# stevenlsw/reart

Measured on AMD Instinct MI355X. Metric: relaxation-loop iterations/sec, higher is better.
Workload: dtype f32; 1 GPU; synthetic T=20 x N=4096, P=20, Chamfer+flow, full iteration, one instance/GPU; frames=20, points=4096, parts=20, flow=True, graph=True, steps_per_graph=20, graph_replays=1, eager_steps=0, parallelism=instances x1, instances_per_gpu=1

## Files before the change

### reart_amd/csrc/prune.hip

```cpp
#include "common.h"
#include "internal.h"
#include <math.h>
#include <string.h>
#include <stddef.h>

typedef float f2 __attribute__((ext_vector_type(2)));
struct SearchHot {
    const float *q, *q_alt, *tsoa, *boxes;
    const int *seed;
    float *pd;
    int *pi;
    unsigned int *cost;
    int P1, Ppad, nqg, P2;
    const int *tlen;
};
static_assert(sizeof(SearchHot) == 88 && offsetof(KnnJob, tlen) == offsetof(SearchHot, tlen) && offsetof(KnnJob, q) == 0 && offsetof(KnnJob, q_alt) == offsetof(SearchHot, q_alt) &&
              offsetof(KnnJob, tsoa) == offsetof(SearchHot, tsoa) && offsetof(KnnJob, boxes) == offsetof(SearchHot, boxes) &&
              offsetof(KnnJob, seed) == offsetof(SearchHot, seed) && offsetof(KnnJob, pd) == offsetof(SearchHot, pd) &&
              offsetof(KnnJob, pi) == offsetof(SearchHot, pi) && offsetof(KnnJob, cost) == offsetof(SearchHot, cost) &&
              offsetof(KnnJob, P1) == offsetof(SearchHot, P1) && offsetof(KnnJob, Ppad) == offsetof(SearchHot, Ppad) &&
              offsetof(KnnJob, nqg) == offsetof(SearchHot, nqg) && offsetof(KnnJob, P2) == offsetof(SearchHot, P2),
              "SearchHot mirrors the head of KnnJob");
__device__ __forceinline__ int pr_uniform_word(const void *p) { return *(const __attribute__((address_space(4))) int *)p; }
#define PR_SMAX 4
#define PR_QCAP 640
#define PR_WPE 6
#define PR_LDS_WAVE_BYTES (64 * 4 + 64 * 16 + 3 * 64 * 8 + PR_QCAP * 4)

#ifdef REART_PRUNE_STATS
__device__ unsigned long long g_prune_stats[8];
extern "C" int reart_debug_prune_stats(unsigned long long *out, int reset) {
    if (hipMemcpyFromSymbol(out, HIP_SYMBOL(g_prune_stats), sizeof(g_prune_stats)) != hipSuccess) return REART_ERR_LAUNCH;
    if (reset) { unsigned long long z[8] = {0}; (void)hipMemcpyToSymbol(HIP_SYMBOL(g_prune_stats), z, sizeof(z)); }
    return REART_OK;
}
#define PRUNE_STAT(k, v) do { if ((threadIdx.x & 63) == 0) atomicAdd(&g_prune_stats[k], (unsigned long long)(v)); } while (0)
#else
#define PRUNE_STAT(k, v) do { } while (0)
#endif
#ifdef REART_PRUNE_PHASE
__device__ unsigned long long g_prune_phase[8];
extern "C" int reart_debug_prune_phase(unsigned long long *out, int reset) {
    if (hipMemcpyFromSymbol(out, HIP_SYMBOL(g_prune_phase), sizeof(g_prune_phase)) != hipSuccess) return REART_ERR_LAUNCH;
    if (reset) { unsigned long long z[8] = {0}; (void)hipMemcpyToSymbol(HIP_SYMBOL(g_prune_phase), z, sizeof(z)); }
    return REART_OK;
}
#define PH_DECL unsigned long long ph_t = __builtin_amdgcn_s_memtime(), ph_acc[7] = {0, 0, 0, 0, 0, 0, 0}
#define PH(k) do { const unsigned long long n_ = __builtin_amdgcn_s_memtime(); ph_acc[k] += n_ - ph_t; ph_t = n_; } while (0)
#define PH_FLUSH(from, to) do { if ((threadIdx.x & 63) == 0) for (int k_ = from; k_ <= to; ++k_) atomicAdd(&g_prune_phase[k_], ph_acc[k_]); } while (0)
__device__ unsigned long long g_prune_head[2][8];
extern "C" int reart_debug_prune_head(unsigned long long *out, int reset) {
    if (hipMemcpyFromSymbol(out, HIP_SYMBOL(g_prune_head), sizeof(g_prune_head)) != hipSuccess) return REART_ERR_LAUNCH;
    if (reset) { unsigned long long z[16] = {0}; (void)hipMemcpyToSymbol(HIP_SYMBOL(g_prune_head), z, sizeof(z)); }
    return REART_OK;
}
#define PH_HEAD_DECL unsigned long long hd_t = ph_t, hd_acc[3] = {0, 0, 0}
#define PH_STAMP(k, ...) do { asm volatile("" :: __VA_ARGS__); const unsigned long long n_ = __builtin_amdgcn_s_memtime(); hd_acc[k] = n_ - hd_t; hd_t = n_; } while (0)
#define PH_HEAD_FLUSH(row) do { if ((threadIdx.x & 63) == 0) { for (int k_ = 0; k_ < 3; ++k_) atomicAdd(&g_prune_head[row][1 + k_], hd_acc[k_]); \
                                atomicAdd(&g_prune_head[row][4], ph_acc[0]); atomicAdd(&g_prune_head[row][6], 1ull); } } while (0)
#define PH_ENTRY const unsigned long long hd_entry = __builtin_amdgcn_s_memtime(); unsigned long long hd_head = 0ull
#define PH_HEAD_END do { hd_head = __builtin_amdgcn_s_memtime() - hd_entry; } while (0)
#define PH_ENTRY_FLUSH(row) do { if ((threadIdx.x & 63) == 0) { atomicAdd(&g_prune_head[row][0], hd_head); \
                                 atomicAdd(&g_prune_head[row][5], __builtin_amdgcn_s_memtime() - hd_entry); } } while (0)
#else
#define PH_DECL do { } while (0)
#define PH(k) do { } while (0)
#define PH_FLUSH(from, to) do { } while (0)
#define PH_HEAD_DECL do { } while (0)
#define PH_STAMP(k, ...) do { } while (0)
#define PH_HEAD_FLUSH(row) do { } while (0)
#define PH_ENTRY do { } while (0)
#define PH_HEAD_END do { } while (0)
#define PH_ENTRY_FLUSH(row) do { } while (0)
#endif

#define PR_WORK(w) ((unsigned)(w) << 20)

#define PR_DPP_OP(NAME, OP, CTRLTXT)                                                                              \
    __device__ __forceinline__ float NAME(float v) {                                                              \
        float r;                                                                                                  \
        asm("s_nop 1\n\t" OP " %0, %1, %1 " CTRLTXT " row_mask:0xf bank_mask:0xf" : "=v"(r) : "v"(v));            \
        return r;                                                                                                 \
    }
PR_DPP_OP(pr_min_q1, "v_min_f32_dpp", "quad_perm:[1,0,3,2]")
PR_DPP_OP(pr_min_q2, "v_min_f32_dpp", "quad_perm:[2,3,0,1]")
PR_DPP_OP(pr_min_hm, "v_min_f32_dpp", "row_half_mirror")
PR_DPP_OP(pr_min_rm, "v_min_f32_dpp", "row_mirror")
PR_DPP_OP(pr_max_q1, "v_max_f32_dpp", "quad_perm:[1,0,3,2]")
PR_DPP_OP(pr_max_q2, "v_max_f32_dpp", "quad_perm:[2,3,0,1]")
PR_DPP_OP(pr_max_hm, "v_max_f32_dpp", "row_half_mirror")
PR_DPP_OP(pr_max_rm, "v_max_f32_dpp", "row_mirror")
__device__ __forceinline__ float pr_row16_min(float v) { return pr_min_rm(pr_min_hm(pr_min_q2(pr_min_q1(v)))); }
__device__ __forceinline__ float pr_row16_max(float v) { return pr_max_rm(pr_max_hm(pr_max_q2(pr_max_q1(v)))); }

__device__ __forceinline__ float rl(float v, int lane) {
    return __int_as_float(__builtin_amdgcn_readlane(__float_as_int(v), lane));
}

__device__ __forceinline__ float box_lb(float lo0, float lo1, float lo2, float hi0, float hi1, float hi2,
                                        float qlo0, float qlo1, float qlo2, float qhi0, float qhi1, float qhi2) {
    const float ex = fmaxf(fmaxf(lo0 - qhi0, qlo0 - hi0), 0.f);
    const float ey = fmaxf(fmaxf(lo1 - qhi1, qlo1 - hi1), 0.f);
    const float ez = fmaxf(fmaxf(lo2 - qhi2, qlo2 - hi2), 0.f);
    return (ex * ex + ey * ey) + ez * ez;
}

template <int KK, bool LDSV, int QCAP, bool BOXL>
__device__ __forceinline__ void knn_pruned_wave(const float *qcloud, const int *seed_p, const int P1, const int n2,
                                                const int S, const int sparse, const int b, const int g,
                                                const int s, const float *cloud, const int cstride, const float *boxes_p,
                                                float *s_tg, float *s_qc, unsigned int *s_q, float *s_bb, const int share, float *s_xthr,
                                                unsigned long long *s_key, float &qx_o, float &qy_o, float &qz_o,
                                                float (&bm)[KK], int (&bb)[KK], int &work_o, unsigned int &pairs_o) {
    struct { int S, sparse; } a = {S, sparse};
    const int lane = threadIdx.x & 63;
    PH_DECL;
    PH_HEAD_DECL;

    const int i = g * NN_BS + lane;
    const int ic = i < P1 ? i : P1 - 1;
    const float *qp = (const float *)((const char *)qcloud + 12u * (unsigned)ic);
    const float qx = qp[0], qy = qp[1], qz = qp[2];
    PH_STAMP(0, "v"(qx), "v"(qy), "v"(qz));
    const f2 qx2 = {qx, qx}, qy2 = {qy, qy}, qz2 = {qz, qz};

    const float *tx = cloud;
    const float *ty = tx + cstride;
    const float *tz = ty + cstride;
    const int nbox = (n2 + NN_BOX - 1) / NN_BOX;
    const float *bx = boxes_p;

    float thr = 0.f;
    unsigned int wp = 0u;
    {
        const int *sd = (const int *)((const char *)(seed_p + (size_t)b * P1 * KK) + 4u * KK * (unsigned)ic);
        int sj[KK];
        bool ok = true;
#pragma unroll
        for (int k = 0; k < KK; ++k) {
            sj[k] = sd[k];
            ok = ok && sj[k] >= 0 && sj[k] < n2;
#pragma unroll
            for (int k2 = 0; k2 < k; ++k2) ok = ok && sj[k] != sj[k2];
        }
        PH_STAMP(1, "v"(sj[0]), "v"(sj[KK - 1]), "s"(n2));
        constexpr bool SCR_JOINT = BOXL;
        constexpr bool SCR_FITS = (384 + QCAP + (SCR_JOINT ? 384 : 0)) >= KK * 3 * 64;
        if (SCR_FITS && share) {
            float *s_scr = (float *)s_key;
            float sx[KK], sy[KK], sz[KK];
#pragma unroll
            for (int k = 0; k < KK; ++k) {
                const int j = ok ? sj[k] : 0;
                sx[k] = tx[j]; sy[k] = ty[j]; sz[k] = tz[j];
            }
            if (!LDSV) __builtin_amdgcn_sched_barrier(0);
#pragma unroll
            for (int k = 0; k < KK; ++k) {
                s_scr[(3 * k + 0) * 64 + lane] = ok ? sx[k] : INFINITY;
                s_scr[(3 * k + 1) * 64 + lane] = ok ? sy[k] : INFINITY;
                s_scr[(3 * k + 2) * 64 + lane] = ok ? sz[k] : INFINITY;
            }
            PH_STAMP(2, "v"(lane));
            thr = INFINITY;
            const float *row = s_scr + (lane & 48);
            const bool split = s_xthr != nullptr && a.S > 1;
            const int c0 = split ? 2 * s : 0, cstep = split ? 2 * a.S : 2;
            wp = 64u * KK * 2u * (unsigned)((16 - c0 + cstep - 1) / cstep);
#pragma unroll 1
            for (int c = c0; c < 16; c += cstep) {
                f2 far = {0.f, 0.f};
#pragma unroll
                for (int k = 0; k < KK; ++k) {
                    const f2 dx = qx2 - *(const f2 *)(row + (3 * k + 0) * 64 + c);
                    const f2 dy = qy2 - *(const f2 *)(row + (3 * k + 1) * 64 + c);
                    const f2 dz = qz2 - *(const f2 *)(row + (3 * k + 2) * 64 + c);
                    const f2 d = (dx * dx + dy * dy) + dz * dz;
                    far = f2{fmaxf(far.x, d.x), fmaxf(far.y, d.y)};
                }
                thr = fminf(thr, fminf(far.x, far.y));
            }
            if (split) {
                s_xthr[64 * s + lane] = thr;
                __syncthreads();
                for (int t = 0; t < a.S; ++t) thr = fminf(thr, s_xthr[64 * t + lane]);
            }
            if (!(qx == qx && qy == qy && qz == qz)) thr = INFINITY;
        } else {
#pragma unroll
            for (int k = 0; k < KK; ++k) {
                const int j = ok ? sj[k] : 0;
                thr = fmaxf(thr, reart_sqdist3(qx, qy, qz, tx[j], ty[j], tz[j]));
            }
            wp = 64u * KK;
            if (!ok || !(thr >= 0.f)) thr = INFINITY;
        }
    }

    const float gl0 = pr_row16_min(qx), gl1 = pr_row16_min(qy), gl2 = pr_row16_min(qz);
    const float gh0 = pr_row16_max(qx), gh1 = pr_row16_max(qy), gh2 = pr_row16_max(qz);
    const float gt = pr_row16_max(thr);
    float G[4][7];
#pragma unroll
    for (int q = 0; q < 4; ++q) {
        G[q][0] = rl(gl0, 16 * q); G[q][1] = rl(gl1, 16 * q); G[q][2] = rl(gl2, 16 * q);
        G[q][3] = rl(gh0, 16 * q); G[q][4] = rl(gh1, 16 * q); G[q][5] = rl(gh2, 16 * q);
        G[q][6] = rl(gt, 16 * q);
    }

#pragma unroll
    for (int k = 0; k < KK; ++k) { bm[k] = INFINITY; bb[k] = -1; }
    const float *tx_g = tx;
    wp |= PR_WORK(16);

    const int queue_max = a.sparse;
    int qcnt = 0;
    ((float4 *)s_qc)[lane] = make_float4(qx, qy, qz, 0.f);
    if (KK == 1) s_key[lane] = ~0ull;
    else { s_key[lane] = ~0ull; s_key[64 + lane] = ~0ull; s_key[128 + lane] = ~0ull; }
    auto drain_queue = [&]() {
        for (int e0 = 0; e0 < qcnt; e0 += 64) {
            wp += PR_WORK(6);
            const int e = e0 + lane;
            const bool valid = e < qcnt;
            const unsigned ent = s_q[valid ? e : e0];
            const int ql = (int)(ent & 63u), j0 = (int)(ent >> 6) * NN_BOX;
            wp += (unsigned)__builtin_popcountll(__ballot(valid)) * NN_BOX;
            const float4 qc = ((const float4 *)s_qc)[ql];
            const float *rx = tx_g, *ry = tx_g + cstride, *rz = tx_g + 2 * (size_t)cstride;
            const f2 cx = {qc.x, qc.x}, cy = {qc.y, qc.y}, cz = {qc.z, qc.z};
            float mh[2] = {INFINITY, INFINITY};
#pragma unroll 1
            for (int hf = 0; hf < 2; ++hf) {
                float4 X[2], Y[2], Z[2];
#pragma unroll
                for (int u = 0; u < 2; ++u) {
                    const unsigned ob = 4u * ((unsigned)j0 + 8u * hf + 4u * u);
                    X[u] = *(const float4 *)((const char *)rx + ob);
                    Y[u] = *(const float4 *)((const char *)ry + ob);
                    Z[u] = *(const float4 *)((const char *)rz + ob);
                }
                float m = INFINITY;
#pragma unroll
                for (int u = 0; u < 2; ++u) {
                    const f2 dxa = cx - f2{X[u].x, X[u].y}, dya = cy - f2{Y[u].x, Y[u].y}, dza = cz - f2{Z[u].x, Z[u].y};
                    const f2 dxb = cx - f2{X[u].z, X[u].w}, dyb = cy - f2{Y[u].z, Y[u].w}, dzb = cz - f2{Z[u].z, Z[u].w};
                    const f2 da = (dxa * dxa + dya * dya) + dza * dza;
                    const f2 db = (dxb * dxb + dyb * dyb) + dzb * dzb;
                    m = fminf(fminf(m, fminf(da.x, da.y)), fminf(db.x, db.y));
                }
                if (hf == 0) mh[0] = m; else mh[1] = m;
            }
            if (KK == 1) {
                const float m = fminf(mh[0], mh[1]);
                const unsigned long long key = ((unsigned long long)__float_as_uint(m) << 32) | (unsigned)(j0 + (mh[1] < mh[0] ? 8 : 0));
                if (valid) atomicMin(&s_key[ql], key);
            } else if (valid) {
#pragma unroll
                for (int h = 0; h < 2; ++h) {
                    unsigned long long key = ((unsigned long long)__float_as_uint(mh[h]) << 32) | (unsigned)(j0 + 8 * h);
#pragma unroll
                    for (int lv = 0; lv < 3; ++lv) {
                        const unsigned long long old = atomicMin(&s_key[64 * lv + ql], key);
                        key = old > key ? old : key;
                    }
                }
            }
        }
        qcnt = 0;
        if (KK == 1) {
            const unsigned long long k = s_key[lane];
            const float m = __uint_as_float((unsigned)(k >> 32));
            const int blk = (int)(unsigned)k;
            if (k != ~0ull && ((m < bm[0]) || (m == bm[0] && blk < bb[0]))) { bm[0] = m; bb[0] = blk; }
            thr = fminf(thr, bm[0]);
            s_key[lane] = ~0ull;
        } else {
            float kd[3];
            int ki[3];
#pragma unroll
            for (int c = 0; c < 3; ++c) { kd[c] = bm[c]; ki[c] = bb[c] >= 0 ? bb[c] : 0x7fffffff; }
#pragma unroll
            for (int c = 0; c < 3; ++c) {
                const unsigned long long k = s_key[64 * c + lane];
                s_key[64 * c + lane] = ~0ull;
                if (k != ~0ull) reart_top3_insert(kd, ki, __uint_as_float((unsigned)(k >> 32)), (int)(unsigned)k);
            }
#pragma unroll
            for (int c = 0; c < 3; ++c) { bm[c] = kd[c]; bb[c] = ki[c] == 0x7fffffff ? -1 : ki[c]; }
            thr = fminf(thr, bm[KK - 1]);
        }
    };
    const int per = 64 * a.S;
    PH(0);
    for (int base = 0; base < nbox; base += per) {
        const int bid = base + lane * a.S + s;
        bool pass = false;
        float lo0 = INFINITY, lo1 = INFINITY, lo2 = INFINITY, hi0 = INFINITY, hi1 = INFINITY, hi2 = INFINITY;
        if (bid < nbox) {
            const float4 A = *(const float4 *)(bx + (size_t)bid * 8);
            const float4 Bv = *(const float4 *)(bx + (size_t)bid * 8 + 4);
            lo0 = A.x; lo1 = A.y; lo2 = A.z; hi0 = A.w; hi1 = Bv.x; hi2 = Bv.y;
            if (BOXL) {
                float *o = s_bb + 6 * lane;
                o[0] = lo0; o[1] = lo1; o[2] = lo2; o[3] = hi0; o[4] = hi1; o[5] = hi2;
            }
            const f2 bl0 = {lo0, lo0}, bl1 = {lo1, lo1}, bl2 = {lo2, lo2}, bh0 = {hi0, hi0}, bh1 = {hi1, hi1}, bh2 = {hi2, hi2};
#pragma unroll
            for (int q = 0; q < 4; q += 2) {
                const f2 ql0 = {G[q][0], G[q + 1][0]}, ql1 = {G[q][1], G[q + 1][1]}, ql2 = {G[q][2], G[q + 1][2]};
                const f2 qh0 = {G[q][3], G[q + 1][3]}, qh1 = {G[q][4], G[q + 1][4]}, qh2 = {G[q][5], G[q + 1][5]};
                const f2 a0 = bl0 - qh0, c0 = ql0 - bh0, a1 = bl1 - qh1, c1 = ql1 - bh1, a2 = bl2 - qh2, c2 = ql2 - bh2;
                const f2 e0 = {fmaxf(fmaxf(a0.x, c0.x), 0.f), fmaxf(fmaxf(a0.y, c0.y), 0.f)};
                const f2 e1 = {fmaxf(fmaxf(a1.x, c1.x), 0.f), fmaxf(fmaxf(a1.y, c1.y), 0.f)};
                const f2 e2 = {fmaxf(fmaxf(a2.x, c2.x), 0.f), fmaxf(fmaxf(a2.y, c2.y), 0.f)};
                const f2 lb = (e0 * e0 + e1 * e1) + e2 * e2;
                pass = pass || (lb.x <= G[q][6]) || (lb.y <= G[q + 1][6]);
            }
        }
        unsigned long long mask = __ballot(pass);
        PH(1);
        PRUNE_STAT(KK == 1 ? 0 : 3, 0);
        if (KK == 1) PRUNE_STAT(1, __builtin_popcountll(mask));
        if (KK == 1) PRUNE_STAT(3, __builtin_popcountll(__ballot(thr == INFINITY)));
        auto scan_box = [&](const int bit) {
            wp += PR_WORK(5) | (64u * NN_BOX);
            if (KK == 1) PRUNE_STAT(2, 1);
            const int j0 = (base + bit * a.S + s) * NN_BOX;
            if (!LDSV) {
                const int l = lane < 48 ? lane : 47;
                const float v = tx_g[(size_t)(l >> 4) * cstride + j0 + (l & 15)];
                if (lane < 48) s_tg[lane] = v;
            }
            const float *tx = LDSV ? tx_g : s_tg - j0;
            const float *ty = tx + (LDSV ? cstride : 16), *tz = ty + (LDSV ? cstride : 16);
            if (KK == 1) {
                float mh[2] = {INFINITY, INFINITY};
#pragma unroll
                for (int u = 0; u < NN_BOX; u += 2) {
                    const f2 dx = qx2 - *(const f2 *)(tx + j0 + u);
                    const f2 dy = qy2 - *(const f2 *)(ty + j0 + u);
                    const f2 dz = qz2 - *(const f2 *)(tz + j0 + u);
                    const f2 d = (dx * dx + dy * dy) + dz * dz;
                    mh[u >> 3] = fminf(fminf(mh[u >> 3], d.x), d.y);
                }
                const float m = fminf(mh[0], mh[1]);
                if (m < bm[0]) { bm[0] = m; bb[0] = j0 + (mh[1] < mh[0] ? 8 : 0); }
                thr = fminf(thr, m);
            } else {
                constexpr int UBK = 8;
#pragma unroll
                for (int h = 0; h < NN_BOX; h += UBK) {
                    float m = INFINITY;
#pragma unroll
                    for (int u = 0; u < UBK; u += 2) {
                        const f2 dx = qx2 - *(const f2 *)(tx + j0 + h + u);
                        const f2 dy = qy2 - *(const f2 *)(ty + j0 + h + u);
                        const f2 dz = qz2 - *(const f2 *)(tz + j0 + h + u);
                        const f2 d = (dx * dx + dy * dy) + dz * dz;
                        m = fminf(fminf(m, d.x), d.y);
                    }
#pragma unroll
                    for (int c = KK - 1; c >= 0; --c) {
                        const int cp = c > 0 ? c - 1 : 0;
                        const bool lt_prev = (c > 0) && (m < bm[cp]);
                        const bool lt_cur = m < bm[c];
                        bm[c] = lt_prev ? bm[cp] : (lt_cur ? m : bm[c]);
                        bb[c] = lt_prev ? bb[cp] : (lt_cur ? j0 + h : bb[c]);
                    }
                }
                thr = fminf(thr, bm[KK - 1]);
            }
        };
        auto enqueue_box = [&](const int bit, const unsigned long long need, const bool nd, const int nneed) {
            wp += PR_WORK(1);
            if (KK == 1) PRUNE_STAT(2, 1);
            const int bid = base + bit * a.S + s;
            const int rank = __builtin_amdgcn_mbcnt_hi((unsigned)(need >> 32), __builtin_amdgcn_mbcnt_lo((unsigned)need, 0u));
            if (nd) s_q[qcnt + rank] = ((unsigned)bid << 6) | (unsigned)lane;
            qcnt += nneed;
        };
        while (mask) {
            unsigned long long cm = mask;
            mask = 0ull;
            while (cm) {
            const int bA = __builtin_ctzll(cm);
            cm &= cm - 1;
            const bool hasB = cm != 0;
            const int bB = hasB ? __builtin_ctzll(cm) : bA;
            if (hasB) cm &= cm - 1;
            f2 L0, L1, L2, H0, H1, H2;
            if (BOXL) {
                const float *pA = s_bb + 6 * bA, *pB = s_bb + 6 * bB;
                L0 = f2{pA[0], pB[0]}; L1 = f2{pA[1], pB[1]}; L2 = f2{pA[2], pB[2]};
                H0 = f2{pA[3], pB[3]}; H1 = f2{pA[4], pB[4]}; H2 = f2{pA[5], pB[5]};
            } else {
                L0 = f2{rl(lo0, bA), rl(lo0, bB)}; L1 = f2{rl(lo1, bA), rl(lo1, bB)}; L2 = f2{rl(lo2, bA), rl(lo2, bB)};
                H0 = f2{rl(hi0, bA), rl(hi0, bB)}; H1 = f2{rl(hi1, bA), rl(hi1, bB)}; H2 = f2{rl(hi2, bA), rl(hi2, bB)};
            }
            const f2 a0 = L0 - qx2, c0 = qx2 - H0, a1 = L1 - qy2, c1 = qy2 - H1, a2 = L2 - qz2, c2 = qz2 - H2;
            const f2 e0 = {fmaxf(fmaxf(a0.x, c0.x), 0.f), fmaxf(fmaxf(a0.y, c0.y), 0.f)};
            const f2 e1 = {fmaxf(fmaxf(a1.x, c1.x), 0.f), fmaxf(fmaxf(a1.y, c1.y), 0.f)};
            const f2 e2 = {fmaxf(fmaxf(a2.x, c2.x), 0.f), fmaxf(fmaxf(a2.y, c2.y), 0.f)};
            const f2 lb = (e0 * e0 + e1 * e1) + e2 * e2;
            wp += PR_WORK(2);
            PH(2);
#pragma unroll 1
            for (int h = 0; h < (hasB ? 2 : 1); ++h) {
                const float lbh = h ? lb.y : lb.x;
#ifdef REART_PRUNE_STATS
                if (KK == 1) {
                    const int nl = __builtin_popcountll(__ballot(lbh <= thr));
                    if (nl) PRUNE_STAT(nl == 1 ? 4 : (nl < 4 ? 5 : (nl < 8 ? 6 : 7)), 1);
                }
#endif
                const bool nd = lbh <= thr;
                const unsigned long long need = __ballot(nd);
                if (need) {
                    const int nneed = __builtin_popcountll(need);
                    if (nneed <= queue_max) {
                        enqueue_box(h ? bB : bA, need, nd, nneed);
                        PH(4);
                        if (qcnt > QCAP - 64) { drain_queue(); PH(5); }
                    } else {
                        scan_box(h ? bB : bA);
                        PH(3);
                    }
                }
            }
            }
        }
    }

    PH(2);
    if (qcnt > 0) drain_queue();
    PH(5);
    PH_FLUSH(0, 5);
    PH_HEAD_FLUSH(KK == 1 ? 0 : 1);
    qx_o = qx; qy_o = qy; qz_o = qz;
    work_o = (int)(wp >> 20); pairs_o = wp & 0xFFFFFu;
}


template <bool BATCH>
__global__ __launch_bounds__(64 * PR_SMAX, PR_WPE) void knn_group_kernel(Batched<SearchArgs> ab) {
    PH_ENTRY;
    const SearchArgs &a_ = ab.a[BATCH ? blockIdx.y : 0];
    extern __shared__ __attribute__((aligned(16))) unsigned char s_dyn[];
#define PARK_M(t) ((float *)(s_dyn + (size_t)(t) * PR_LDS_WAVE_BYTES + 64 * 4 + 64 * 16))
#define PARK_B(t) ((int *)(s_dyn + (size_t)(t) * PR_LDS_WAVE_BYTES + 64 * 4 + 64 * 16 + 3 * 64 * 4))
    __shared__ unsigned int s_wk[PR_SMAX][2];
    __shared__ float s_xthr[PR_SMAX][64];
    __shared__ unsigned int s_ticket;
    __shared__ unsigned long long s_t0;
    struct { int n1, n3, G, per, S1, S3, interleave, sparse; } a = {a_.n1, a_.n3, a_.G, a_.per, a_.S1, a_.S3, a_.interleave, a_.sparse};
    const unsigned int *const items = a_.item;
    unsigned long long *const prof = a_.prof;
    const int share = a_.share;
    asm volatile("" :: "s"(a.n1), "s"(a.n3), "s"(a.G), "s"(a.per), "s"(a.S1), "s"(a.S3), "s"(a.interleave), "s"(a.sparse), "s"(items), "s"(prof), "s"(share));
    const int L = blockIdx.x, x = L & 7, r = L >> 3;
    const int s = threadIdx.x >> 6, lane = threadIdx.x & 63;
    const int items1 = a.n1 * a.per, items3 = a.n3 * a.per;
    const int mixed = (a.n1 == 2 && a.n3) ? 3 * a.per : 0;
    int kind, idx;
    if (r < mixed) {
        const int q = r / 3, rr = r - 3 * q;
        kind = rr < 2 ? 1 : 3;
        idx = rr < 2 ? 2 * q + rr : q;
    } else {
        const int d1 = mixed ? 2 * a.per : 0, d3 = mixed ? a.per : 0;
        const int v = r - mixed, left1 = items1 - d1;
        kind = v < left1 ? 1 : 3;
        idx = v < left1 ? d1 + v : d3 + (v - left1);
    }
    const int j = kind == 1 ? (a.n1 == 2 ? (idx & 1) : 0) : 0;
    const int p = kind == 1 ? (a.n1 == 2 ? (idx >> 1) : idx) : idx;
    const int pos = a.interleave ? p * 8 + x : x * a.per + p;
    const bool live = p < a.per && pos < a.G && (kind == 1 ? idx < items1 : idx < items3);
    const KnnJob *jp = kind == 1 ? &a_.k1[j] : &a_.k3;
    int rec = pos;
    if (items) rec = pr_uniform_word(items + ((size_t)(kind == 1 ? j : 2) * a.G + (live ? pos : 0)));
    SearchHot h;
    __builtin_memcpy(&h, jp, sizeof(SearchHot));
    if (threadIdx.x == 0) { s_ticket = 0u; s_t0 = prof ? wall_clock64() : 0ull; }
    __syncthreads();
    asm volatile("" :: "s"(rec), "s"(h.tlen), "s"(h.q), "s"(h.q_alt), "s"(h.tsoa), "s"(h.boxes), "s"(h.seed), "s"(h.pd),
                 "s"(h.pi), "s"(h.cost), "s"(h.P1), "s"(h.Ppad), "s"(h.nqg), "s"(h.P2));
    const unsigned long long t0 = s_t0;
    if (!live) {
        if (prof && threadIdx.x == 0) { prof[2 * (size_t)L] = t0; prof[2 * (size_t)L + 1] = t0; a_.prof_pairs[L] = 0u; }
        return;
    }
    const int S = kind == 1 ? a.S1 : a.S3;
    if (s >= S) return;
    const int grp = items ? (int)((unsigned)rec & SEARCH_ITEM_PAIR_MASK) : (jp->border ? jp->border[pos] : pos);
    const int b = grp / h.nqg, g = grp - b * h.nqg;
    const int qb = items ? (int)((unsigned)rec >> SEARCH_ITEM_PAIR_BITS) - 1 : (jp->qmap ? jp->qmap[b] : b);
    const int n2 = h.tlen ? pr_uniform_word(h.tlen + b) : h.P2;
    const float *qcloud = qb < 0 ? h.q_alt : h.q + (size_t)qb * h.P1 * 3;
    float qx = 0.f, qy = 0.f, qz = 0.f;
    float bm[3] = {INFINITY, INFINITY, INFINITY};
    int bb[3] = {-1, -1, -1};
    int work = 0;
    unsigned int pairs = 0u;
    {
        unsigned char *wl = s_dyn + (size_t)s * PR_LDS_WAVE_BYTES;
        float *s_tg = (float *)wl;
        float *s_qc = (float *)(wl + 64 * 4);
        unsigned long long *s_key = (unsigned long long *)(wl + 64 * 4 + 64 * 16);
        unsigned int *s_q = (unsigned int *)(wl + 64 * 4 + 64 * 16 + 3 * 64 * 8);
        static_assert(384 + PR_QCAP >= 3 * 3 * 64, "neighbour seeds of a K = 3 item: 9 x 64 floats in the result slots + the queue's space");
        static_assert(PR_QCAP >= 384 + 128, "box bounds of a coarse round + at least two drain steps of queue");
        float *s_bb = (float *)s_q;
        s_q += 384;
        constexpr int QC = PR_QCAP - 384;
        const float *cloud = h.tsoa + (size_t)b * 3 * h.Ppad;
        const float *boxes_p = h.boxes + (size_t)b * (h.Ppad / NN_BOX) * 8;
        PH_HEAD_END;
        if (kind == 1) {
            float m1[1]; int b1[1];
            knn_pruned_wave<1, false, QC, true>(qcloud, h.seed, h.P1, n2, S, a.sparse, b, g, s, cloud, h.Ppad, boxes_p, s_tg, s_qc, s_q, s_bb, share, share > 1 ? &s_xthr[0][0] : nullptr, s_key,
                                               qx, qy, qz, m1, b1, work, pairs);
            bm[0] = m1[0]; bb[0] = b1[0];
        } else {
            knn_pruned_wave<3, false, QC, true>(qcloud, h.seed, h.P1, n2, S, a.sparse, b, g, s, cloud, h.Ppad, boxes_p, s_tg, s_qc, s_q, s_bb, share, share > 1 ? &s_xthr[0][0] : nullptr, s_key,
                                               qx, qy, qz, bm, bb, work, pairs);
        }
        PH_ENTRY_FLUSH(kind == 1 ? 0 : 1);
    }
    if (S > 1) {
#pragma unroll
        for (int k = 0; k < 3; ++k) { PARK_M(s)[k * 64 + lane] = bm[k]; PARK_B(s)[k * 64 + lane] = bb[k]; }
        if (lane == 0) { s_wk[s][0] = (unsigned int)work; s_wk[s][1] = pairs; }
        __threadfence_block();
        int ticket = 0;
        if (lane == 0) ticket = (int)atomicAdd(&s_ticket, 1u);
        ticket = __builtin_amdgcn_readfirstlane(ticket);
#ifdef REART_PRUNE_PHASE
        if (lane == 0) atomicAdd(&g_prune_phase[7], 1ull);
#endif
        if (ticket != S - 1) return;
        __threadfence_block();
        work = 0; pairs = 0u;
        for (int t = 0; t < S; ++t) { work += (int)s_wk[t][0]; pairs += s_wk[t][1]; }
#pragma unroll
        for (int k = 0; k < 3; ++k) { bm[k] = PARK_M(0)[k * 64 + lane]; bb[k] = PARK_B(0)[k * 64 + lane]; }
    }
    const int i = g * NN_BS + lane;
    const float *tx = h.tsoa + (size_t)b * 3 * h.Ppad, *ty = tx + h.Ppad, *tz = ty + h.Ppad;
    if (kind == 1) {
        float m = bm[0];
        int blk = bb[0];
        for (int t = 1; t < S; ++t) {
            const float mt = PARK_M(t)[lane];
            const int bt = PARK_B(t)[lane];
            const bool take = bt >= 0 && ((mt < m) || (mt == m && (blk < 0 || bt < blk)));
            m = take ? mt : m; blk = take ? bt : blk;
        }
        int bi = 0x7fffffff;
        if (blk >= 0) {
#pragma unroll
            for (int u = NN_BOX / 2 - 1; u >= 0; --u) {
                const float d = reart_sqdist3(qx, qy, qz, tx[blk + u], ty[blk + u], tz[blk + u]);
                if (d == m) bi = blk + u;
            }
        }
        pairs += 64u * (NN_BOX / 2);
        if (i < h.P1) {
            const size_t o = (size_t)b * h.P1 + i;
            h.pd[o] = m; h.pi[o] = bi;
        }
    } else {
        float kd[3] = {INFINITY, INFINITY, INFINITY};
        int ki[3] = {0x7fffffff, 0x7fffffff, 0x7fffffff};
#pragma unroll
        for (int k = 0; k < 3; ++k) reart_top3_insert(kd, ki, bm[k], bb[k] >= 0 ? bb[k] : 0x7fffffff);
        for (int t = 1; t < S; ++t) {
#pragma unroll
            for (int k = 0; k < 3; ++k) {
                const int bt = PARK_B(t)[k * 64 + lane];
                reart_top3_insert(kd, ki, PARK_M(t)[k * 64 + lane], bt >= 0 ? bt : 0x7fffffff);
            }
        }
        if (i < h.P1) {
            const size_t o = ((size_t)b * h.P1 + i) * 3;
#pragma unroll
            for (int k = 0; k < 3; ++k) { h.pd[o + k] = kd[k]; h.pi[o + k] = kd[k] < INFINITY ? ki[k] : -1; }
        }
    }
    if (lane == 0) {
        if (h.cost) h.cost[pos] = (unsigned int)work;
        if (prof) {
            prof[2 * (size_t)L] = t0; prof[2 * (size_t)L + 1] = wall_clock64();
            a_.prof_pairs[L] = pairs;
        }
    }
}

#define PC_WAVES 16
#define PC_QCAP 256
#define PC_WAVE_BYTES (64 * 16 + 3 * 64 * 8 + PC_QCAP * 4)
__global__ __launch_bounds__(64 * PC_WAVES) void knn_cloud_kernel(SearchArgs a) {
    extern __shared__ __attribute__((aligned(16))) unsigned char s_dyn[];
    const int L = blockIdx.x, w = threadIdx.x >> 6, lane = threadIdx.x & 63;
    unsigned long long t0 = 0ull;
    if (a.prof && threadIdx.x == 0) t0 = wall_clock64();
    const int njobs = a.n1 + a.n3;
    const int jsel = L % njobs;
    const int rest = L / njobs;
    const int B = a.G / a.k_nqg;
    const int b = rest % B, blk = rest / B;
    const int kind = jsel < a.n1 ? 1 : 3;
    const KnnJob &jb = kind == 1 ? a.k1[jsel] : a.k3;
    const int S = a.cloud_slices, gpw = PC_WAVES / S;
    const int Ppad = jb.Ppad, nboxp = Ppad / NN_BOX;
    float *cl = (float *)s_dyn;
    float *bxs = cl + 3 * (size_t)Ppad;
    {
        const float4 *src = (const float4 *)(jb.tsoa + (size_t)b * 3 * Ppad);
        float4 *dst = (float4 *)cl;
        const int n4 = 3 * Ppad / 4;
        for (int e = threadIdx.x; e < n4; e += 64 * PC_WAVES) dst[e] = src[e];
        const float4 *sb = (const float4 *)(jb.boxes + (size_t)b * nboxp * 8);
        float4 *db = (float4 *)bxs;
        for (int e = threadIdx.x; e < 2 * nboxp; e += 64 * PC_WAVES) db[e] = sb[e];
    }
    __syncthreads();
    const int g = blk * gpw + w / S, sl = w % S;
    unsigned int pairs = 0u;
    int work = 0;
    unsigned char *wbase = s_dyn + (size_t)(3 * Ppad + 8 * nboxp) * 4;
    unsigned long long *s_key = (unsigned long long *)(wbase + (size_t)w * PC_WAVE_BYTES + 64 * 16);
    float qx = 0.f, qy = 0.f, qz = 0.f;
    float bm[3] = {INFINITY, INFINITY, INFINITY};
    int bb[3] = {-1, -1, -1};
    if (g < jb.nqg) {
        unsigned char *wl = wbase + (size_t)w * PC_WAVE_BYTES;
        float *s_qc = (float *)wl;
        unsigned int *s_q = (unsigned int *)(wl + 64 * 16 + 3 * 64 * 8);
        const int qb = jb.qmap ? jb.qmap[b] : b;
        const float *qcloud = qb < 0 ? jb.q_alt : jb.q + (size_t)qb * jb.P1 * 3;
        const int n2 = jb.tlen ? jb.tlen[b] : jb.P2;
        if (kind == 1) {
            float m1[1]; int b1[1];
            knn_pruned_wave<1, true, PC_QCAP, false>(qcloud, jb.seed, jb.P1, n2, S, a.sparse, b, g, sl, cl, Ppad, bxs, nullptr, s_qc, s_q, nullptr, a.share, nullptr, s_key, qx, qy, qz,
                                              m1, b1, work, pairs);
            bm[0] = m1[0]; bb[0] = b1[0];
        } else {
            knn_pruned_wave<3, true, PC_QCAP, false>(qcloud, jb.seed, jb.P1, n2, S, a.sparse, b, g, sl, cl, Ppad, bxs, nullptr, s_qc, s_q, nullptr, a.share, nullptr, s_key, qx, qy, qz,
                                              bm, bb, work, pairs);
        }
        if (S > 1 && sl > 0) {
#pragma unroll
            for (int k = 0; k < 3; ++k)
                s_key[64 * k + lane] = bb[k] >= 0 ? (((unsigned long long)__float_as_uint(bm[k]) << 32) | (unsigned)bb[k]) : ~0ull;
            if (lane == 0) { s_key[192] = (unsigned long long)(unsigned)work; s_key[193] = (unsigned long long)pairs; }
        }
    }
    if (S > 1) __syncthreads();
    if (g < jb.nqg && sl == 0) {
        for (int t = 1; t < S; ++t) {
            const unsigned long long *ok = (const unsigned long long *)(wbase + (size_t)(w + t) * PC_WAVE_BYTES + 64 * 16);
            work += (int)(unsigned)ok[192]; pairs += (unsigned)ok[193];
            if (kind == 1) {
                const unsigned long long k = ok[lane];
                const float m = __uint_as_float((unsigned)(k >> 32));
                const int bt = (int)(unsigned)k;
                if (k != ~0ull && ((m < bm[0]) || (m == bm[0] && (bb[0] < 0 || bt < bb[0])))) { bm[0] = m; bb[0] = bt; }
            } else {
                float kd[3];
                int ki[3];
#pragma unroll
                for (int c = 0; c < 3; ++c) { kd[c] = bm[c]; ki[c] = bb[c] >= 0 ? bb[c] : 0x7fffffff; }
#pragma unroll
                for (int c = 0; c < 3; ++c) {
                    const unsigned long long k = ok[64 * c + lane];
                    if (k != ~0ull) reart_top3_insert(kd, ki, __uint_as_float((unsigned)(k >> 32)), (int)(unsigned)k);
                }
#pragma unroll
                for (int c = 0; c < 3; ++c) { bm[c] = kd[c]; bb[c] = ki[c] == 0x7fffffff ? -1 : ki[c]; }
            }
        }
        const int i = g * NN_BS + lane;
        if (kind == 1) {
            int bi = 0x7fffffff;
            if (bb[0] >= 0) {
                const float *tx = cl, *ty = cl + Ppad, *tz = cl + 2 * (size_t)Ppad;
#pragma unroll
                for (int u = NN_BOX / 2 - 1; u >= 0; --u) {
                    const float d = reart_sqdist3(qx, qy, qz, tx[bb[0] + u], ty[bb[0] + u], tz[bb[0] + u]);
                    if (d == bm[0]) bi = bb[0] + u;
                }
            }
            pairs += 64u * (NN_BOX / 2);
            if (i < jb.P1) {
                const size_t o = (size_t)b * jb.P1 + i;
                jb.pd[o] = bm[0]; jb.pi[o] = bi;
            }
        } else if (i < jb.P1) {
            const size_t o = ((size_t)b * jb.P1 + i) * 3;
#pragma unroll
            for (int k = 0; k < 3; ++k) { jb.pd[o + k] = bm[k]; jb.pi[o + k] = bm[k] < INFINITY ? bb[k] : -1; }
        }
        if (lane == 0 && jb.cost) jb.cost[b * jb.nqg + g] = (unsigned int)work;
    } else {
        pairs = 0u;
    }
    if (a.prof) {
        __shared__ unsigned int s_pairs[PC_WAVES];
        if (lane == 0) s_pairs[w] = pairs;
        __syncthreads();
        if (threadIdx.x == 0) {
            unsigned int tot = 0u;
            for (int k = 0; k < PC_WAVES; ++k) tot += s_pairs[k];
            a.prof[2 * (size_t)L] = t0; a.prof[2 * (size_t)L + 1] = wall_clock64();
            a.prof_pairs[L] = tot;
        }
    }
}

static size_t search_cloud_lds(const SearchArgs &a) {
    int Ppad = 0;
    for (int j = 0; j < a.n1; ++j) Ppad = a.k1[j].Ppad > Ppad ? a.k1[j].Ppad : Ppad;
    if (a.n3) Ppad = a.k3.Ppad > Ppad ? a.k3.Ppad : Ppad;
    const size_t need = (size_t)(3 * Ppad + 8 * (Ppad / NN_BOX)) * 4 + (size_t)PC_WAVES * PC_WAVE_BYTES + 256;
    return need <= 152 * 1024 ? need : 0;
}

static int search_check(SearchArgs &a) {
    if (a.n1 < 0 || a.n1 > 2 || a.n3 < 0 || a.n3 > 1 || a.n1 + a.n3 == 0 || a.G < 1) return REART_ERR_INVALID_ARG;
    if ((a.n1 && (a.S1 < 1 || a.S1 > PR_SMAX)) || (a.n3 && (a.S3 < 1 || a.S3 > PR_SMAX))) return REART_ERR_INVALID_ARG;
    for (int j = 0; j < a.n1; ++j)
        if (!a.k1[j].boxes || !a.k1[j].seed || !a.k1[j].pd || !a.k1[j].pi) return REART_ERR_INVALID_ARG;
    if (a.n3 && (!a.k3.boxes || !a.k3.seed || !a.k3.pd || !a.k3.pi)) return REART_ERR_INVALID_ARG;
    a.per = reart_div_up(a.G, 8);
    a.k_nqg = a.n1 ? a.k1[0].nqg : a.k3.nqg;
    return REART_OK;
}

int reart_search_launch(const SearchArgs &a_in, hipStream_t st) {
    SearchArgs a = a_in;
    const int rc = search_check(a);
    if (rc != REART_OK) return rc;
    const size_t cl_lds = a.cloud_resident ? search_cloud_lds(a) : 0;
    a.cloud_slices = (a.cloud_slices == 1 || a.cloud_slices == 2 || a.cloud_slices == 4 || a.cloud_slices == 8) ? a.cloud_slices : 4;
    if (cl_lds) {
        if (hipFuncSetAttribute((const void *)knn_cloud_kernel, hipFuncAttributeMaxDynamicSharedMemorySize, 152 * 1024) != hipSuccess)
            return REART_ERR_LAUNCH;
        hipLaunchKernelGGL(knn_cloud_kernel, dim3(reart_search_grid_cloud(a.n1, a.n3, a.G, a.k_nqg, a.cloud_slices)), dim3(64 * PC_WAVES),
                           cl_lds, st, a);
        REART_CHECK_LAUNCH();
        return REART_OK;
    }
    return reart_search_launch_batch(&a, 1, st);
}
int reart_search_launch_batch(const SearchArgs *ak, int K, hipStream_t st) {
    if (K < 1 || K > REART_BATCH_MAX) return REART_ERR_INVALID_ARG;
    Batched<SearchArgs> ab = {};
    for (int k = 0; k < K; ++k) {
        ab.a[k] = ak[k];
        const int rc = search_check(ab.a[k]);
        if (rc != REART_OK) return rc;
        const SearchArgs &a = ab.a[k], &a0 = ab.a[0];
        if (a.n1 != a0.n1 || a.n3 != a0.n3 || a.G != a0.G || a.S1 != a0.S1 || a.S3 != a0.S3) return REART_ERR_INVALID_ARG;
    }
    const SearchArgs &a = ab.a[0];
    const int S = (a.n1 ? a.S1 : 0) > (a.n3 ? a.S3 : 0) ? a.S1 : a.S3;
    const size_t lds = (size_t)S * PR_LDS_WAVE_BYTES;
    if (K == 1) hipLaunchKernelGGL(knn_group_kernel<false>, dim3(reart_search_grid(a.n1, a.n3, a.G)), dim3(64 * S), lds, st, ab);
    else hipLaunchKernelGGL(knn_group_kernel<true>, dim3(reart_search_grid(a.n1, a.n3, a.G), K), dim3(64 * S), lds, st, ab);
    REART_CHECK_LAUNCH();
    return REART_OK;
}
int reart_search_workgroups(const SearchArgs &a) {
    const int nqg = a.n1 ? a.k1[0].nqg : a.k3.nqg;
    const int cs = (a.cloud_slices == 1 || a.cloud_slices == 2 || a.cloud_slices == 4 || a.cloud_slices == 8) ? a.cloud_slices : 4;
    if (a.cloud_resident && search_cloud_lds(a)) return reart_search_grid_cloud(a.n1, a.n3, a.G, nqg, cs);
    return reart_search_grid(a.n1, a.n3, a.G);
}
int reart_search_grid(int n1, int n3, int G) { return 8 * (n1 + n3) * reart_div_up(G, 8); }
int reart_search_grid_cloud(int n1, int n3, int G, int nqg, int slices) {
    return (n1 + n3) * (G / nqg) * reart_div_up(nqg, PC_WAVES / slices);
}

template <int KK>
__global__ __launch_bounds__(256) void knn_warm_finish_kernel(KnnArgs a) {
    const KnnJob jb = a.job[0];
    const int b = blockIdx.y, i = blockIdx.x * 256 + threadIdx.x;
    if (i >= jb.P1) return;
    float kd[KK];
    int ki[KK];
#pragma unroll
    for (int k = 0; k < KK; ++k) { kd[k] = INFINITY; ki[k] = 0x7fffffff; }
    auto insert = [&](float d, int j) {
#pragma unroll
        for (int s = KK - 1; s >= 0; --s) {
            const int sp = s > 0 ? s - 1 : 0;
            const bool lp = (s > 0) && ((d < kd[sp]) | ((d == kd[sp]) & (j < ki[sp])));
            const bool lc = (d < kd[s]) | ((d == kd[s]) & (j < ki[s]));
            kd[s] = lp ? kd[sp] : (lc ? d : kd[s]);
            ki[s] = lp ? ki[sp] : (lc ? j : ki[s]);
        }
    };
    {
        const size_t o = ((size_t)b * jb.P1 + i) * KK;
#pragma unroll
        for (int k = 0; k < KK; ++k) {
            const float d = jb.pd[o + k];
            const int q = jb.pi[o + k];
            insert(d, (d < INFINITY && q >= 0) ? q : 0x7fffffff);
        }
    }
    if (KK > 1) {
        const float *qp = jb.q + ((size_t)b * jb.P1 + i) * 3;
        const float qx = qp[0], qy = qp[1], qz = qp[2];
        const float *tx = jb.tsoa + (size_t)b * 3 * jb.Ppad, *ty = tx + jb.Ppad, *tz = ty + jb.Ppad;
        int blk[KK];
#pragma unroll
        for (int k = 0; k < KK; ++k) { blk[k] = kd[k] < INFINITY ? ki[k] : -1; kd[k] = INFINITY; ki[k] = 0x7fffffff; }
#pragma unroll
        for (int c = 0; c < KK; ++c) {
            if (blk[c] < 0) continue;
            for (int u = 0; u < 8; ++u) {
                const int jj = blk[c] + u;
                const float d = reart_sqdist3(qx, qy, qz, tx[jj], ty[jj], tz[jj]);
                insert(d, d < INFINITY ? jj : 0x7fffffff);
            }
        }
    }
    const int n2 = jb.P2;
    const int valid = KK < n2 ? KK : n2;
#pragma unroll
    for (int k = 0; k < KK; ++k) {
        const bool ok = k < valid && ki[k] != 0x7fffffff;
        const size_t o = ((size_t)b * jb.P1 + i) * KK + k;
        jb.dists[o] = ok ? kd[k] : 0.0f;
        jb.idx[o] = ok ? (int64_t)ki[k] : (int64_t)0;
        ((int *)jb.seed)[o] = ok ? ki[k] : -1;
    }
}

struct WarmPlan { int S, Ppad; size_t o_soa, o_box, o_pd, o_pi, total; };
static int warm_plan(int N, int P1, int P2, int K, WarmPlan *p) {
    if (N < 0 || P1 < 0 || P2 < 0 || (K != 1 && K != 3)) return REART_ERR_INVALID_ARG;
    p->S = 4;
    while (p->S > 1 && reart_div_up(P2, p->S) < 64) p->S -= 1;
    p->Ppad = (int)reart_align_up((size_t)(P2 > 0 ? P2 : 1), NN_BOX);
    reart_arena ws;
    p->o_soa = ws.take_bytes(sizeof(float) * 3 * (size_t)N * p->Ppad);
    p->o_box = ws.take_bytes(sizeof(float) * 8 * (size_t)N * (p->Ppad / NN_BOX));
    p->o_pd = ws.take_bytes(sizeof(float) * (size_t)N * P1 * K);
    p->o_pi = ws.take_bytes(sizeof(int) * (size_t)N * P1 * K);
    p->total = ws.off;
    return REART_OK;
}

extern "C" size_t reart_knn_points_warm_workspace_bytes(int N, int P1, int P2, int K) {
    WarmPlan p;
    return warm_plan(N, P1, P2, K, &p) == REART_OK ? p.total : 0;
}

extern "C" int reart_knn_points_idx_warm(const float *p1, const float *p2, int N, int P1, int P2, int K,
                                         int32_t *seed, float *dists, int64_t *idx, void *workspace,
                                         size_t workspace_bytes, void *stream) {
    WarmPlan p;
    int rc = warm_plan(N, P1, P2, K, &p);
    if (rc != REART_OK) return rc;
    if (N == 0 || P1 == 0) return REART_OK;
    if (!p1 || !p2 || !seed || !dists || !idx || P2 < 1) return REART_ERR_INVALID_ARG;
    if (!workspace || workspace_bytes < p.total) return REART_ERR_INVALID_ARG;
    hipStream_t st = (hipStream_t)stream;
    char *ws = (char *)workspace;
    SoaArgs sa = {};
    for (int j = 0; j < 2; ++j) {
        sa.job[j].src = p2; sa.job[j].len = nullptr; sa.job[j].dst = (float *)(ws + p.o_soa);
        sa.job[j].P = P2; sa.job[j].Ppad = p.Ppad;
    }
    rc = reart_soa_launch(sa, p.Ppad, N, 1, st);
    if (rc != REART_OK) return rc;
    rc = reart_boxes_launch((const float *)(ws + p.o_soa), N, p.Ppad, (float *)(ws + p.o_box), st);
    if (rc != REART_OK) return rc;
    KnnArgs a = {};
    a.N = N; a.S = p.S; a.K = K; a.euclidean = 0;
    KnnJob &jb = a.job[0];
    jb.q = p1; jb.tsoa = (const float *)(ws + p.o_soa); jb.boxes = (const float *)(ws + p.o_box);
    jb.seed = seed; jb.P1 = P1; jb.P2 = P2; jb.Ppad = p.Ppad; jb.L = 0; jb.nqg = reart_div_up(P1, NN_BS);
    jb.pd = (float *)(ws + p.o_pd); jb.pi = (int *)(ws + p.o_pi); jb.dists = dists; jb.idx = idx;
    a.job[1] = jb;
    SearchArgs sr = {};
    sr.G = N * jb.nqg; sr.S1 = sr.S3 = p.S; sr.sparse = 40; sr.share = 2;
    if (K == 1) { sr.k1[0] = jb; sr.n1 = 1; } else { sr.k3 = jb; sr.n3 = 1; }
    rc = reart_search_launch(sr, st);
    if (rc != REART_OK) return rc;
    const dim3 fg(reart_div_up(P1, 256), N);
    if (K == 1) hipLaunchKernelGGL((knn_warm_finish_kernel<1>), fg, dim3(256), 0, st, a);
    else hipLaunchKernelGGL((knn_warm_finish_kernel<3>), fg, dim3(256), 0, st, a);
    REART_CHECK_LAUNCH();
    return REART_OK;
}
```

Baseline: 13850 iterations/s.

## Restructure box-pruning loop with deferred rare paths and packed LDS bounds

Rewrites the inner box-selection loop so the rare scan_box and queue-drain paths leave the hot loop: the loop records the pending box and remaining mask, exits, handles the slow path, then resumes. The per-lane box bounds in LDS are reordered (x/y lo, x/y hi, z lo, negated z hi) so they load as packed float2 pairs and the lower-bound test uses fewer ops. The change also swaps launch_bounds occupancy for an explicit waves_per_eu attribute, forces the wave index scalar with readfirstlane, and pins the queue offset in an SGPR. Debug event counters are added under the stats macro. Together these aim to cut VGPR pressure and divergent control flow in the hottest loop, at the cost of more complex loop state.

```diff
diff --git a/reart_amd/csrc/prune.hip b/reart_amd/csrc/prune.hip
--- a/reart_amd/csrc/prune.hip
+++ b/reart_amd/csrc/prune.hip
@@ -35,8 +35,16 @@
     return REART_OK;
 }
 #define PRUNE_STAT(k, v) do { if ((threadIdx.x & 63) == 0) atomicAdd(&g_prune_stats[k], (unsigned long long)(v)); } while (0)
+__device__ unsigned long long g_prune_events[2][8];
+extern "C" int reart_debug_prune_events(unsigned long long *out, int reset) {
+    if (hipMemcpyFromSymbol(out, HIP_SYMBOL(g_prune_events), sizeof(g_prune_events)) != hipSuccess) return REART_ERR_LAUNCH;
+    if (reset) { unsigned long long z[16] = {0}; (void)hipMemcpyToSymbol(HIP_SYMBOL(g_prune_events), z, sizeof(z)); }
+    return REART_OK;
+}
+#define PRUNE_EVENT(k, v) do { if ((threadIdx.x & 63) == 0) atomicAdd(&g_prune_events[KK == 1 ? 0 : 1][k], (unsigned long long)(v)); } while (0)
 #else
 #define PRUNE_STAT(k, v) do { } while (0)
+#define PRUNE_EVENT(k, v) do { } while (0)
 #endif
 #ifdef REART_PRUNE_PHASE
 __device__ unsigned long long g_prune_phase[8];
@@ -123,6 +131,7 @@
     const float qx = qp[0], qy = qp[1], qz = qp[2];
     PH_STAMP(0, "v"(qx), "v"(qy), "v"(qz));
     const f2 qx2 = {qx, qx}, qy2 = {qy, qy}, qz2 = {qz, qz};
+    const f2 qxy = {qx, qy}, qzn = {-qz, qz};
 
     const float *tx = cloud;
     const float *ty = tx + cstride;
@@ -221,6 +230,7 @@
     auto drain_queue = [&]() {
         for (int e0 = 0; e0 < qcnt; e0 += 64) {
             wp += PR_WORK(6);
+            PRUNE_EVENT(6, 1);
             const int e = e0 + lane;
             const bool valid = e < qcnt;
             const unsigned ent = s_q[valid ? e : e0];
@@ -303,7 +313,7 @@
             lo0 = A.x; lo1 = A.y; lo2 = A.z; hi0 = A.w; hi1 = Bv.x; hi2 = Bv.y;
             if (BOXL) {
                 float *o = s_bb + 6 * lane;
-                o[0] = lo0; o[1] = lo1; o[2] = lo2; o[3] = hi0; o[4] = hi1; o[5] = hi2;
+                o[0] = lo0; o[1] = lo1; o[2] = hi0; o[3] = hi1; o[4] = lo2; o[5] = -hi2;
             }
             const f2 bl0 = {lo0, lo0}, bl1 = {lo1, lo1}, bl2 = {lo2, lo2}, bh0 = {hi0, hi0}, bh1 = {hi1, hi1}, bh2 = {hi2, hi2};
 #pragma unroll
@@ -315,17 +325,20 @@
                 const f2 e1 = {fmaxf(fmaxf(a1.x, c1.x), 0.f), fmaxf(fmaxf(a1.y, c1.y), 0.f)};
                 const f2 e2 = {fmaxf(fmaxf(a2.x, c2.x), 0.f), fmaxf(fmaxf(a2.y, c2.y), 0.f)};
                 const f2 lb = (e0 * e0 + e1 * e1) + e2 * e2;
-                pass = pass || (lb.x <= G[q][6]) || (lb.y <= G[q + 1][6]);
+                pass = pass | (lb.x <= G[q][6]) | (lb.y <= G[q + 1][6]);
             }
         }
         unsigned long long mask = __ballot(pass);
         PH(1);
         PRUNE_STAT(KK == 1 ? 0 : 3, 0);
+        PRUNE_EVENT(0, 1);
+        PRUNE_EVENT(1, __builtin_popcountll(mask));
         if (KK == 1) PRUNE_STAT(1, __builtin_popcountll(mask));
         if (KK == 1) PRUNE_STAT(3, __builtin_popcountll(__ballot(thr == INFINITY)));
         auto scan_box = [&](const int bit) {
             wp += PR_WORK(5) | (64u * NN_BOX);
             if (KK == 1) PRUNE_STAT(2, 1);
+            PRUNE_EVENT(5, 1);
             const int j0 = (base + bit * a.S + s) * NN_BOX;
             if (!LDSV) {
                 const int l = lane < 48 ? lane : 47;
@@ -375,63 +388,84 @@
         auto enqueue_box = [&](const int bit, const unsigned long long need, const bool nd, const int nneed) {
             wp += PR_WORK(1);
             if (KK == 1) PRUNE_STAT(2, 1);
+            PRUNE_EVENT(4, 1);
             const int bid = base + bit * a.S + s;
             const int rank = __builtin_amdgcn_mbcnt_hi((unsigned)(need >> 32), __builtin_amdgcn_mbcnt_lo((unsigned)need, 0u));
             if (nd) s_q[qcnt + rank] = ((unsigned)bid << 6) | (unsigned)lane;
             qcnt += nneed;
         };
-        while (mask) {
-            unsigned long long cm = mask;
-            mask = 0ull;
-            while (cm) {
-            const int bA = __builtin_ctzll(cm);
-            cm &= cm - 1;
-            const bool hasB = cm != 0;
-            const int bB = hasB ? __builtin_ctzll(cm) : bA;
-            if (hasB) cm &= cm - 1;
-            f2 L0, L1, L2, H0, H1, H2;
-            if (BOXL) {
-                const float *pA = s_bb + 6 * bA, *pB = s_bb + 6 * bB;
-                L0 = f2{pA[0], pB[0]}; L1 = f2{pA[1], pB[1]}; L2 = f2{pA[2], pB[2]};
-                H0 = f2{pA[3], pB[3]}; H1 = f2{pA[4], pB[4]}; H2 = f2{pA[5], pB[5]};
-            } else {
-                L0 = f2{rl(lo0, bA), rl(lo0, bB)}; L1 = f2{rl(lo1, bA), rl(lo1, bB)}; L2 = f2{rl(lo2, bA), rl(lo2, bB)};
-                H0 = f2{rl(hi0, bA), rl(hi0, bB)}; H1 = f2{rl(hi1, bA), rl(hi1, bB)}; H2 = f2{rl(hi2, bA), rl(hi2, bB)};
-            }
-            const f2 a0 = L0 - qx2, c0 = qx2 - H0, a1 = L1 - qy2, c1 = qy2 - H1, a2 = L2 - qz2, c2 = qz2 - H2;
-            const f2 e0 = {fmaxf(fmaxf(a0.x, c0.x), 0.f), fmaxf(fmaxf(a0.y, c0.y), 0.f)};
-            const f2 e1 = {fmaxf(fmaxf(a1.x, c1.x), 0.f), fmaxf(fmaxf(a1.y, c1.y), 0.f)};
-            const f2 e2 = {fmaxf(fmaxf(a2.x, c2.x), 0.f), fmaxf(fmaxf(a2.y, c2.y), 0.f)};
-            const f2 lb = (e0 * e0 + e1 * e1) + e2 * e2;
-            wp += PR_WORK(2);
-            PH(2);
-#pragma unroll 1
-            for (int h = 0; h < (hasB ? 2 : 1); ++h) {
-                const float lbh = h ? lb.y : lb.x;
+        wp += PR_WORK(2 * ((__builtin_popcountll(mask) + 1) >> 1));
+#define PR_NEEDED_BOX(BIT, NEED, ND)                                                                              \
+        PRUNE_EVENT(3, 1);                                                                                        \
+        const int nneed = __builtin_popcountll(NEED);                                                             \
+        if (nneed > queue_max) { rare = (BIT); left = cm; cm = 0ull; }                                            \
+        else { enqueue_box((BIT), (NEED), (ND), nneed); PH(4);                                                    \
+               if (qcnt > QCAP - 64) { rare = -2; left = cm; cm = 0ull; } }
+        unsigned long long cm = mask;
+        for (;;) {
+            int rare = -1;
+            unsigned long long left = 0ull;
+            while (cm != 0) {
+                const int bA = __builtin_ctzll(cm);
+                const unsigned long long restA = cm & (cm - 1);
+                const bool hasB = restA != 0;
+                const int bB = hasB ? __builtin_ctzll(restA) : bA;
+                f2 lb;
+                if constexpr (BOXL) {
+                    const f2 *pA = (const f2 *)(s_bb + 6 * bA), *pB = (const f2 *)(s_bb + 6 * bB);
+                    const f2 LA = pA[0], HA = pA[1], ZA = pA[2];
+                    const f2 LB = pB[0], HB = pB[1], ZB = pB[2];
+                    const f2 aA = LA - qxy, cA = qxy - HA, zA = ZA + qzn;
+                    const f2 aB = LB - qxy, cB = qxy - HB, zB = ZB + qzn;
+                    const f2 eA = {fmaxf(fmaxf(aA.x, cA.x), 0.f), fmaxf(fmaxf(aA.y, cA.y), 0.f)};
+                    const f2 eB = {fmaxf(fmaxf(aB.x, cB.x), 0.f), fmaxf(fmaxf(aB.y, cB.y), 0.f)};
+                    const f2 ez = {fmaxf(fmaxf(zA.x, zA.y), 0.f), fmaxf(fmaxf(zB.x, zB.y), 0.f)};
+                    const f2 sA = eA * eA, sB = eB * eB;
+                    float tA = sA.x + sA.y, tB = sB.x + sB.y;
+                    asm("" : "+v"(tA), "+v"(tB));
+                    lb = f2{tA, tB} + ez * ez;
+                } else {
+                    const f2 L0 = f2{rl(lo0, bA), rl(lo0, bB)}, L1 = f2{rl(lo1, bA), rl(lo1, bB)}, L2 = f2{rl(lo2, bA), rl(lo2, bB)};
+                    const f2 H0 = f2{rl(hi0, bA), rl(hi0, bB)}, H1 = f2{rl(hi1, bA), rl(hi1, bB)}, H2 = f2{rl(hi2, bA), rl(hi2, bB)};
+                    const f2 a0 = L0 - qx2, c0 = qx2 - H0, a1 = L1 - qy2, c1 = qy2 - H1, a2 = L2 - qz2, c2 = qz2 - H2;
+                    const f2 e0 = {fmaxf(fmaxf(a0.x, c0.x), 0.f), fmaxf(fmaxf(a0.y, c0.y), 0.f)};
+                    const f2 e1 = {fmaxf(fmaxf(a1.x, c1.x), 0.f), fmaxf(fmaxf(a1.y, c1.y), 0.f)};
+                    const f2 e2 = {fmaxf(fmaxf(a2.x, c2.x), 0.f), fmaxf(fmaxf(a2.y, c2.y), 0.f)};
+                    lb = (e0 * e0 + e1 * e1) + e2 * e2;
+                }
+                PRUNE_EVENT(2, 1);
+                PH(2);
 #ifdef REART_PRUNE_STATS
                 if (KK == 1) {
-                    const int nl = __builtin_popcountll(__ballot(lbh <= thr));
+                    const int nl = __builtin_popcountll(__ballot(lb.x <= thr));
                     if (nl) PRUNE_STAT(nl == 1 ? 4 : (nl < 4 ? 5 : (nl < 8 ? 6 : 7)), 1);
                 }
 #endif
-                const bool nd = lbh <= thr;
-                const unsigned long long need = __ballot(nd);
-                if (need) {
-                    const int nneed = __builtin_popcountll(need);
-                    if (nneed <= queue_max) {
-                        enqueue_box(h ? bB : bA, need, nd, nneed);
-                        PH(4);
-                        if (qcnt > QCAP - 64) { drain_queue(); PH(5); }
-                    } else {
-                        scan_box(h ? bB : bA);
-                        PH(3);
-                    }
-                }
-            }
-            }
-        }
-    }
-
+                cm = restA;
+                const bool ndA = lb.x <= thr;
+                const unsigned long long needA = __ballot(ndA);
+                if (needA) { PR_NEEDED_BOX(bA, needA, ndA) }
+                if (cm == 0) continue;
+                cm = restA & (restA - 1);
+#ifdef REART_PRUNE_STATS
+                if (KK == 1) {
+                    const int nl = __builtin_popcountll(__ballot(lb.y <= thr));
+                    if (nl) PRUNE_STAT(nl == 1 ? 4 : (nl < 4 ? 5 : (nl < 8 ? 6 : 7)), 1);
+                }
+#endif
+                const bool ndB = lb.y <= thr;
+                const unsigned long long needB = __ballot(ndB);
+                if (needB) { PR_NEEDED_BOX(bB, needB, ndB) }
+            }
+            if (rare == -1) break;
+            if (rare >= 0) { scan_box(rare); PH(3); }
+            else { drain_queue(); PH(5); }
+            cm = left;
+        }
+#undef PR_NEEDED_BOX
+    }
+
+    PRUNE_EVENT(7, 1);
     PH(2);
     if (qcnt > 0) drain_queue();
     PH(5);
@@ -443,7 +477,7 @@
 
 
 template <bool BATCH>
-__global__ __launch_bounds__(64 * PR_SMAX, PR_WPE) void knn_group_kernel(Batched<SearchArgs> ab) {
+__global__ __launch_bounds__(64 * PR_SMAX) __attribute__((amdgpu_waves_per_eu(PR_WPE, PR_WPE))) void knn_group_kernel(Batched<SearchArgs> ab) {
     PH_ENTRY;
     const SearchArgs &a_ = ab.a[BATCH ? blockIdx.y : 0];
     extern __shared__ __attribute__((aligned(16))) unsigned char s_dyn[];
@@ -459,7 +493,7 @@
     const int share = a_.share;
     asm volatile("" :: "s"(a.n1), "s"(a.n3), "s"(a.G), "s"(a.per), "s"(a.S1), "s"(a.S3), "s"(a.interleave), "s"(a.sparse), "s"(items), "s"(prof), "s"(share));
     const int L = blockIdx.x, x = L & 7, r = L >> 3;
-    const int s = threadIdx.x >> 6, lane = threadIdx.x & 63;
+    const int s = __builtin_amdgcn_readfirstlane(threadIdx.x >> 6), lane = threadIdx.x & 63;
     const int items1 = a.n1 * a.per, items3 = a.n3 * a.per;
     const int mixed = (a.n1 == 2 && a.n3) ? 3 * a.per : 0;
     int kind, idx;
@@ -508,7 +542,9 @@
         float *s_tg = (float *)wl;
         float *s_qc = (float *)(wl + 64 * 4);
         unsigned long long *s_key = (unsigned long long *)(wl + 64 * 4 + 64 * 16);
-        unsigned int *s_q = (unsigned int *)(wl + 64 * 4 + 64 * 16 + 3 * 64 * 8);
+        int q_off = s * PR_LDS_WAVE_BYTES + (64 * 4 + 64 * 16 + 3 * 64 * 8);
+        asm("" : "+s"(q_off));
+        unsigned int *s_q = (unsigned int *)(s_dyn + q_off);
         static_assert(384 + PR_QCAP >= 3 * 3 * 64, "neighbour seeds of a K = 3 item: 9 x 64 floats in the result slots + the queue's space");
         static_assert(PR_QCAP >= 384 + 128, "box bounds of a coarse round + at least two drain steps of queue");
         float *s_bb = (float *)s_q;
```

Measured after the change: 14510 iterations/s (median of 6 runs). 1.05x the previous value.
